# angelocatalani/neural-network-compression

Hardware: AMD Instinct MI355X
Metric: weights/sec through prune+k-means (K=256) (higher is better)
Workload: dtype f32

## Files before the change

neural_network_compression_amd/csrc/nnc_hip.hip:

```cpp
#include "nnc_common.hpp"
#include "nnc_km_shared.hpp"


extern "C" size_t nnc_kmeans_workspace_bytes(int32_t k)
{
    (void)k;
    return sizeof(KmWs) + 256;
}

extern "C" int32_t nnc_fix_shift(float absmax, int64_t n_total)
{
    int L = 1;
    while (((int64_t)1 << L) < n_total && L < 62) L++;
    if (!(absmax > 0.0f) || !std::isfinite(absmax)) return 0;
    int P = 0;
    (void)std::frexp((double)absmax, &P);
    return std::min(28, 62 - L) - P;
}

__device__ __forceinline__ int fix_f32(float v, int Sft)
{
    return (int)rintf(ldexpf(v, Sft));
}

// ... 1156 lines not shown
    if (NNC_FIN_TRACE_PTR && tid == 0) {
        unsigned long long *rt = NNC_FIN_TRACE_PTR;
        const int it = min(ws->st.iter, 63);
        rt[300 + 4 * it] = (unsigned long long)hd->n_empty; rt[301 + 4 * it] = (unsigned long long)hd->nch; rt[302 + 4 * it] = (unsigned long long)hd->slow; rt[303 + 4 * it] = (unsigned long long)ku;
    }
    if (hd->slow || hd->nch > 1024) return 0;
    if constexpr (MASS) {
        if (mass) {
            __shared__ KlMass mass_s;
            return kl_relocate_mass<NT>(xs, n, ws, hd, L, &mass_s, sum_o, cnt_o, k, hd->nch, mean, Sft);
        }
    }
    return kl_relocate<NT>(xs, n, ws, hd, L, sum_o, cnt_o, k, hd->nch, mean, Sft);
}

template <int NT, bool ONEWAVE, bool MASS = false>
__device__ __forceinline__ bool km_finalize_body(KmWs *__restrict__ ws, int mode, int resume, int *gcell, int *hcell, int *ku_out, const bool lazy = false,
                                                 const float *__restrict__ reloc_xs = nullptr, const long long reloc_n = 0, const int k_hint = 0)
{
    static_assert(!ONEWAVE || NT == 64, "the barrier-free form is for a single wave");
#define FIN_SYNC() do { if (ONEWAVE) wave_lds_fence(); else km_lds_barrier(); } while (0)
#define FIN_OR(slot, x) (ONEWAVE ? (int)__any(x) : km_vote_or(&fin_votes[slot], (x)))
#define FIN_AND(slot, x) (ONEWAVE ? (int)__all(x) : !km_vote_or(&fin_votes[slot], !(x)))
#define FIN_COUNT(slot, x) (ONEWAVE ? (int)__popcll(__ballot(x)) : km_vote_count(&fin_votes[slot], (x)))
    __shared__ int fin_votes[8];
    __shared__ long long sum_o[NNC_KMAX];
    __shared__ long long cnt_o[NNC_KMAX];
    __shared__ __align__(16) float cnew[NNC_KMAX];
    __shared__ float cs[NNC_KMAX];
    __shared__ uint16_t so[NNC_KMAX];
    __shared__ float sq[NNC_KMAX];
    __shared__ unsigned long long sh_key;
    __shared__ int ovf_n;
// ... 143 lines not shown
            if (n_empty > 0 && (MASS || n_empty <= KL_RM_MAX) && !resume && reloc_xs && mode == FIN_FROM_SHARDS && lazy && !(st_iter >= 1 && same_counts_now)) {
                __syncthreads();
                if (ftr && tid == 0) { ftr[20] = ftr[0]; ftr[21] = __builtin_amdgcn_s_memrealtime(); }
                const KmTab *tabc = &ws->tab[cur];
                settled = km_finalize_relocate<NT, MASS>(ws, reloc_xs, reloc_n, tabc, cur ? ku1 : ku0, k, cur, sum_o, cnt_o, ws->p.x_mean, Sft) != 0;
                if (settled) { n_empty = 0; settled_event = true; }
                if (settled && ftr && tid == 0) ftr[22] = __builtin_amdgcn_s_memrealtime();
            }
        }
        if (n_empty > 0 && !resume) {
            int tot_empty = 0;
            if (tid == 0) {
                for (int j = 0; j < k; j++) tot_empty += (cnt_o[j] == 0);
                ws->st.paused = 1; ws->st.n_empty = tot_empty;
                if (lazy) ws->tab[cur].n_ovf = 0;
            }
            return false;
        }
        for (int j = tid; j < k; j += NT)
            if (cnt_o[j] > 0) cnew[j] = (float)ldexp((double)sum_o[j] / (double)cnt_o[j], -Sft);
        FIN_SYNC();
        if (n_empty > 0) {
            for (int j = tid; j < k; j += NT)
                atomicMax(&sh_key, ((unsigned long long)cnt_o[j] << 11) | (unsigned long long)(2047 - j));
            FIN_SYNC();
            const int amax = 2047 - (int)(sh_key & 2047ull);
            for (int j = tid; j < k; j += NT)
                if (cnt_o[j] <= 0) {
                    cnew[j] = (amax < j) ? cnew[amax] : (float)ldexp((double)sum_o[amax], -Sft);
                }
// ... 272 lines not shown
    int c = hi_p - lo_p;
    int field = lo_p;
    if (c >= KM_CNT_SAT) {
        c = KM_CNT_SAT;
        const int idx = atomicAdd(n_ovf, 1);
        if (idx < KM_OVF_MAX) { ovf[idx] = (unsigned)lo_p | ((unsigned)hi_p << 16); field = idx; }
        else field = (int)KM_OVF_ALL;
    }
    return (uint16_t)(field | (c << KM_P_BITS));
}

template <int NT, bool FUSED, bool MASS = false>
__device__ __forceinline__ void km_finalize_kernel(KmWs *__restrict__ ws, int mode, int resume,
                                                   nnc_kmeans_status *host_st, unsigned long long *host_ticket,
                                                   unsigned long long ticket, int lazy, const float *__restrict__ reloc_xs,
                                                   long long reloc_n)
{
    __shared__ int gcell[NNC_KMAX], hcell[NNC_KMAX];
    __shared__ int fin_go, fin_kc[2], fin_novf;
    __shared__ int fin_asked;
    const int tid = threadIdx.x;
    const int cond = lazy & 2;
    const int k_hint = lazy >> 8;
    lazy &= 1;
    if (cond) {
        if (tid == 0) fin_asked = ws->wide;
        __syncthreads();
    }
    if (cond && !fin_asked) {
    } else if (FUSED) {
        const int glog2 = ws->glog2;
// ... 1 lines not shown
        __syncthreads();
        if (tid < NT) {
            const bool built = km_finalize_body<NT, FUSED>(ws, mode, resume, gcell, hcell, fin_kc, lazy != 0, reloc_xs, reloc_n, k_hint);
            if (tid == 0) __hip_atomic_store(&fin_go, (built && !lazy) ? 1 : 2, __ATOMIC_RELEASE, __HIP_MEMORY_SCOPE_WORKGROUP);
        }
        int go;
        while ((go = __hip_atomic_load(&fin_go, __ATOMIC_ACQUIRE, __HIP_MEMORY_SCOPE_WORKGROUP)) == 0) __builtin_amdgcn_s_sleep(1);
        if (go == 1) {
            KmTab *tab = &ws->tab[fin_kc[1]];
            const int G = 1 << glog2, ku = fin_kc[0];
            for (int g = tid; g < G; g += KM_THREADS) tab->cell[g] = km_cell_entry(g, G, ku, gcell, hcell, &fin_novf, tab->ovf);
            __syncthreads();
            if (tid == 0) tab->n_ovf = fin_novf;
        }
    } else {
        km_finalize_body<NT, false, MASS>(ws, mode, resume, gcell, hcell, fin_kc, lazy != 0, reloc_xs, reloc_n, k_hint);
    }
    if (cond && fin_asked) {
        __syncthreads();
        if (tid == 0) { ws->wide = 0; ws->kl_budget = ws->kl_budget - 1; ws->kl_stats[4] += 1; }
    }
    if (host_st) {
        __syncthreads();
        if (tid == 0) {
            *host_st = ws->st;
            __threadfence_system();
            *reinterpret_cast<volatile unsigned long long *>(host_ticket) = ticket;
        }
    }
}

template <int NT, bool FUSED, bool MASS = false>
__global__ __launch_bounds__(FUSED ? KM_THREADS : NT) void k_finalize(KmWs *__restrict__ ws, int mode, int resume,
                                                                      nnc_kmeans_status *host_st, unsigned long long *host_ticket,
                                                                      unsigned long long ticket, int lazy, const float *__restrict__ reloc_xs,
                                                                      long long reloc_n)
{
    km_finalize_kernel<NT, FUSED, MASS>(ws, mode, resume, host_st, host_ticket, ticket, lazy, reloc_xs, reloc_n);
}

__global__ __launch_bounds__(KM_THREADS) void k_fit_small(const float *__restrict__ xs, long long n, KmWs *__restrict__ ws,
                                                         const long long *__restrict__ pblk, int iters, nnc_kmeans_status *host_st,
                                                         unsigned long long *host_ticket, unsigned long long ticket)
{
    __shared__ int gcell[NNC_KMAX], hcell[NNC_KMAX];
    __shared__ int fin_kc[2];
    const int tid = threadIdx.x, lane = tid & 63, wv = uni_i(tid >> 6);
    const float mean = ws->p.x_mean;
    const int Sft = ws->p.fix_shift;
    for (int it = 0; it < iters; it++) {
        if (ws->st.done | ws->st.paused) break;
        const KmTab *tab = &ws->tab[ws->cur];
        const int ku = ws->bnd.ku;
// ... 103 lines not shown
    return p->prefix_dev && p->n > 0 && p->n == p->n_total && km_fused(p) && (reinterpret_cast<uintptr_t>(x) & 15) == 0;
}

static int km_ensure_cells(KmWs *w, const nnc_kmeans_params *p, int which, void *stream)
{
    if (!p->prefix_dev) return NNC_OK;
    hipLaunchKernelGGL(k_cells_prepare, dim3(1), dim3(1), 0, S(stream), w, which);
    LAUNCHCHK("k_cells_prepare");
    hipLaunchKernelGGL(k_cells, dim3(KM_GMAX / KM_THREADS), dim3(KM_THREADS), 0, S(stream), w, (nnc_kmeans_status *)nullptr,
                       (unsigned long long *)nullptr, 0ull, 1, which);
    LAUNCHCHK("k_cells");
    return NNC_OK;
}

int km_launch_finalize(KmWs *w, const nnc_kmeans_params *p, int mode, int resume, void *stream, void *host_mapped,
                       uint64_t ticket, bool cond, const float *reloc_xs)
{
    const int k = p ? p->k : 0;
    bool fused = false;
    if (p && mode != FIN_PACK_ONLY) fused = km_fused(p);
    const bool lazy = p && p->prefix_dev;
    const bool cells = mode != FIN_PACK_ONLY && !fused && !lazy;
    unsigned char *hb = reinterpret_cast<unsigned char *>(host_mapped);
    nnc_kmeans_status *hs = reinterpret_cast<nnc_kmeans_status *>(hb);
    unsigned long long *ht = reinterpret_cast<unsigned long long *>(hb ? hb + sizeof(nnc_kmeans_status) : nullptr);
    nnc_kmeans_status *fs = cells ? nullptr : hs;
#define KM_LAUNCH_FIN(NT, FUSED, THREADS) NNC_LAUNCH_PROF(NNC_PROF_FINALIZE, (k_finalize<NT, FUSED>), dim3(1), dim3(THREADS), 0, S(stream), w, mode, resume, fs, ht, (unsigned long long)ticket, (lazy ? 1 : 0) | (cond ? 2 : 0) | (k > 0 ? k << 8 : 0), reloc_xs, (long long)(p ? p->n : 0))
#define KM_LAUNCH_FIN_MASS(NT, THREADS) NNC_LAUNCH_PROF(NNC_PROF_FINALIZE, (k_finalize<NT, false, true>), dim3(1), dim3(THREADS), 0, S(stream), w, mode, resume, fs, ht, (unsigned long long)ticket, (lazy ? 1 : 0) | (cond ? 2 : 0) | (k > 0 ? k << 8 : 0), reloc_xs, (long long)(p ? p->n : 0))
    const bool mass = p && (p->flags & NNC_KM_MASS_IN_PLACE) && reloc_xs && !fused && k > 64;
    if (fused) KM_LAUNCH_FIN(64, true, KM_THREADS);
    else if (k > 0 && k <= 64) KM_LAUNCH_FIN(64, false, 64);
    else if (k > 0 && k <= 256) { if (mass) KM_LAUNCH_FIN_MASS(256, 256); else KM_LAUNCH_FIN(256, false, 256); }
    else { if (mass) KM_LAUNCH_FIN_MASS(KM_THREADS, KM_THREADS); else KM_LAUNCH_FIN(KM_THREADS, false, KM_THREADS); }
#undef KM_LAUNCH_FIN_MASS
#undef KM_LAUNCH_FIN
    LAUNCHCHK("k_finalize");
    if (cells) {
        hipLaunchKernelGGL(k_cells, dim3(KM_GMAX / KM_THREADS), dim3(KM_THREADS), 0, S(stream), w, hs, ht, (unsigned long long)ticket, 0, 0);
        LAUNCHCHK("k_cells");
    }
    return NNC_OK;
}

// ... 719 lines not shown
    km_relocate_body(ws, keys, nkeys, &lds);
}

extern "C" int nnc_kmeans_relocate(void *ws, const int64_t *keys_sorted_dev, int32_t nkeys, void *stream)
{
    if (!ws || !keys_sorted_dev || nkeys < 0) return fail(NNC_EINVAL, "nnc_kmeans_relocate: bad argument");
    if (nkeys == 0) return NNC_OK;
    hipLaunchKernelGGL(k_relocate, dim3(1), dim3(KM_THREADS), 0, S(stream), reinterpret_cast<KmWs *>(ws),
                       reinterpret_cast<const long long *>(keys_sorted_dev), nkeys);
    LAUNCHCHK("k_relocate");
    return NNC_OK;
}

struct KmWin { long long start; int len; int off; };

template <bool MAXOP>
__device__ __forceinline__ void block_scan2(long long &a0, long long &a1, long long *wave_tot)
{
    const int tid = threadIdx.x, lane = tid & 63, wv = tid >> 6;
    auto op = [](long long x, long long y) -> long long { return MAXOP ? (x > y ? x : y) : x + y; };
    a1 = op(a0, a1);
    long long s = a1;
    for (int off = 1; off < 64; off <<= 1) {
        const long long t = __shfl_up(s, off);
        if (lane >= off) s = op(s, t);
    }
    if (lane == 63) wave_tot[wv] = s;
    __syncthreads();
    long long pre = 0;
    for (int w = 0; w < wv; w++) pre = op(pre, wave_tot[w]);
// ... 9 lines not shown
#define KM_RELOC_WMIN 64
#endif
#define KM_SURV_MAX 2048
#define KM_SURV_SMALL 384

__device__ __forceinline__ bool km_spec_decide(const KmWs *__restrict__ ws, long long n, int spec_wmax, int *W_out)
{
    const int done = ws->st.done, paused = ws->st.paused, it = ws->st.iter, same = ws->st.same_counts, ne = ws->st.n_empty;
    long long w = KM_RELOC_WMIN;
    while (w < ne) w *= 2;
    if (W_out) *W_out = (int)w;
    return !done && paused == 1 && !(it >= 1 && same) && ne >= 1 && w <= spec_wmax && 2 * w <= n;
}

__device__ __forceinline__ void km_reloc_windows_body(const float *__restrict__ xs, long long n, KmWs *__restrict__ ws, int W, long long cap,
                                                      KmWin *__restrict__ win, int *__restrict__ meta, unsigned *__restrict__ hist0, int spec_wmax)
{
    if (spec_wmax > 0) {
        const bool go = km_spec_decide(ws, n, spec_wmax, &W);
        if (threadIdx.x == 0) ws->spec_go = go ? 1 : 0;
        if (!go) return;
    }
    if (hist0) for (int i = threadIdx.x; i < 4096; i += KM_THREADS) hist0[i] = 0u;
    __shared__ long long bnd[2 * KM_THREADS + 2];
    __shared__ long long wst[2 * KM_THREADS], wen[2 * KM_THREADS];
    __shared__ long long wave_tot[KM_THREADS / 64];
    const int tid = threadIdx.x;
    const KmTab *tab = &ws->tab[ws->cur];
    const int kt = tab->ku, k = ws->p.k;
    const float mean = ws->p.x_mean;
    const int i0 = 2 * tid, i1 = 2 * tid + 1;
    long long a0 = (i0 < kt) ? ws->partials_local[k + tab->orig[i0]] : 0;
    long long a1 = (i1 < kt) ? ws->partials_local[k + tab->orig[i1]] : 0;
    block_scan2<false>(a0, a1, wave_tot);
    if (tid == 0) bnd[0] = 0;
    bnd[i0 + 1] = a0; bnd[i1 + 1] = a1;
    __syncthreads();
    const int nwin = kt + 1;
    const int bad = (bnd[kt] != n) ? 1 : 0;
    if (bad) {
        for (int j = tid; j < nwin; j += KM_THREADS) { KmWin w; w.start = 0; w.len = 0; w.off = 0; win[j] = w; }
        if (tid == 0) { meta[0] = 0; meta[1] = nwin; meta[2] = 1; meta[3] = W; }
        return;
    }
    for (int j = tid; j < 2 * KM_THREADS; j += KM_THREADS) {
        long long st = 0, en = 0;
        if (j < nwin) {
            long long b = bnd[j];
// ... 27 lines not shown
    const long long len0 = l0, len1 = l1;
    block_scan2<false>(l0, l1, wave_tot);
    if (i0 < nwin) { KmWin w; w.start = s0; w.len = (int)len0; w.off = l0 <= cap ? (int)(l0 - len0) : 0; win[i0] = w; }
    if (i1 < nwin) { KmWin w; w.start = s1; w.len = (int)len1; w.off = l1 <= cap ? (int)(l1 - len1) : 0; win[i1] = w; }
    if (tid == (nwin - 1) / 2) {
        const long long total = ((nwin - 1) & 1) ? l1 : l0;
        const int over = total > cap ? 1 : 0;
        meta[0] = over ? 0 : (int)total; meta[1] = nwin; meta[2] = bad | over; meta[3] = W;
    }
}

__global__ __launch_bounds__(KM_THREADS) void k_reloc_windows(const float *__restrict__ xs, long long n, KmWs *__restrict__ ws,
                                                              int W, long long cap, KmWin *__restrict__ win, int *__restrict__ meta,
                                                              unsigned *__restrict__ hist0 = nullptr, int spec_wmax = 0)
{
    if (spec_wmax > 0 && threadIdx.x == 0 && km_spec_decide(ws, n, spec_wmax, nullptr)) ws->tab[ws->cur].n_ovf = 0;
    km_reloc_windows_body(xs, n, ws, W, cap, win, meta, hist0, spec_wmax);
}

__global__ __launch_bounds__(KM_THREADS) void k_reloc_head(const float *__restrict__ xs, long long n, KmWs *__restrict__ ws, long long cap,
                                                           KmWin *__restrict__ win, int *__restrict__ meta, unsigned *__restrict__ hist0, int spec_wmax)
{
    if (blockIdx.x == gridDim.x - 1) {
        km_reloc_windows_body(xs, n, ws, 0, cap, win, meta, hist0, spec_wmax);
    } else {
        if (!km_spec_decide(ws, n, spec_wmax, nullptr)) return;
        km_cells_body(ws, nullptr, nullptr, 0ull, 1, 0, 0, (int)blockIdx.x);
    }
}

__global__ __launch_bounds__(256) void k_reloc_fill(const float *__restrict__ xs, const KmWin *__restrict__ win,
                                                    const int *__restrict__ meta, float *__restrict__ cand_x, long long cap)
{
    const int lane = threadIdx.x & 63;
    const int wave = (int)((blockIdx.x * blockDim.x + threadIdx.x) >> 6), nwaves = (int)((gridDim.x * blockDim.x) >> 6);
    const int nwin = meta[1];
    const long long total = meta[0];
    if (!meta[2])
        for (int j = wave; j < nwin; j += nwaves) {
            const KmWin w = win[j];
            for (int i = lane; i < w.len; i += 64) cand_x[w.off + i] = xs[w.start + i];
        }
    if (blockIdx.x == 0 && threadIdx.x < 4 && total + threadIdx.x < cap) cand_x[total + threadIdx.x] = 0.0f;
}

__global__ __launch_bounds__(KM_THREADS) void k_reloc_dist(const float *__restrict__ xs, const KmWin *__restrict__ win,
                                                           const int *__restrict__ meta, float *__restrict__ cand_x,
                                                           float *__restrict__ cand_d, long long cap, const KmWs *__restrict__ ws,
                                                           unsigned *__restrict__ hist0, int spec = 0)
{
    extern __shared__ __align__(16) unsigned char smem[];
    __shared__ unsigned h0_s[4096];
    if (spec && !ws->spec_go) return;
    for (int i = threadIdx.x; i < 4096; i += KM_THREADS) h0_s[i] = 0u;
    if (meta[2]) {
        if (blockIdx.x == 0 && threadIdx.x < 4 && threadIdx.x < cap) { cand_x[threadIdx.x] = 0.0f; cand_d[threadIdx.x] = 0.0f; }
        return;
    }
    const int k = ws->p.k, glog2 = ws->glog2;
    const int G = 1 << glog2, kp = (k + 7) & ~7;
    const KmTab *__restrict__ tab = &ws->tab[ws->cur];
    const int kt = tab->ku;
    uint16_t *cell_s = reinterpret_cast<uint16_t *>(smem);
    float4 *pair_s = reinterpret_cast<float4 *>(smem + ((size_t)2 << glog2));
    float *cval_s = reinterpret_cast<float *>(smem + ((size_t)2 << glog2) + (size_t)kp * 16);
    uint16_t *orig_s = reinterpret_cast<uint16_t *>(smem + ((size_t)2 << glog2) + (size_t)kp * 20);
    const size_t off = (((size_t)2 << glog2) + (size_t)kp * 22 + 15) & ~(size_t)15;
    unsigned *ovf_s = reinterpret_cast<unsigned *>(smem + off);
    {
        const uint4 *src = reinterpret_cast<const uint4 *>(tab->cell);
        uint4 *dst = reinterpret_cast<uint4 *>(cell_s);
        for (int i = threadIdx.x; i < (G >> 3); i += KM_THREADS) dst[i] = src[i];
        for (int i = threadIdx.x; i < kt; i += KM_THREADS) {
            const float2 a = tab->cand[i];
            const float2 b = (i + 1 < kt) ? tab->cand[i + 1] : a;
            pair_s[i] = make_float4(a.x, a.y, b.x, b.y);
            cval_s[i] = a.x;
            orig_s[i] = tab->orig[i];
        }
        const int novf = min(tab->n_ovf, KM_OVF_MAX);
        for (int i = threadIdx.x; i < novf; i += KM_THREADS) ovf_s[i] = tab->ovf[i];
    }
    __syncthreads();
    KmCtx c;
    c.cell_s = cell_s; c.pair_s = pair_s; c.cval_s = cval_s; c.orig_s = orig_s; c.ovf_s = ovf_s; c.sum_s = nullptr; c.cnt_s = nullptr;
    c.mean = ws->p.x_mean; c.lo = ws->p.lo; c.inv = ws->inv;
    c.Sft = ws->p.fix_shift; c.gmax = G - 1; c.k = kt; c.rlog2 = 0; c.rep = 0;
    const int nwin = meta[1];
    const long long total = meta[0];
    int *woff_s = reinterpret_cast<int *>(smem + off + KM_OVF_MAX * 4);
    for (int j = threadIdx.x; j < nwin; j += KM_THREADS) woff_s[j] = win[j].off;
    __syncthreads();
    for (long long i = (long long)blockIdx.x * KM_THREADS + threadIdx.x; i < total; i += (long long)gridDim.x * KM_THREADS) {
        int l = 0, h = nwin - 1;
        while (l < h) { const int m = (l + h + 1) >> 1; if (woff_s[m] <= (int)i) l = m; else h = m - 1; }
        KmWin w = win[l];
        while (w.len == 0 || (int)i - w.off >= w.len) { l--; w = win[l]; }
        const float xv[1] = {xs[w.start + ((int)i - w.off)]};
        float xc[1];
        int p[1];
        km_resolve<1>(c, xv, xc, p);
        const float dd = xc[0] - cval_s[p[0]];
        const float dv = dd * dd;
        cand_x[i] = xv[0];
        cand_d[i] = dv;
        atomicAdd(&h0_s[(__float_as_uint(dv) >> 19) & 4095u], 1u);
    }
    __syncthreads();
    for (int i = threadIdx.x; i < 4096; i += KM_THREADS)
        if (h0_s[i]) atomicAdd(&hist0[i], h0_s[i]);
    if (blockIdx.x == 0 && threadIdx.x < 4 && total + threadIdx.x < cap) { cand_x[total + threadIdx.x] = 0.0f; cand_d[total + threadIdx.x] = 0.0f; }
}

__device__ __forceinline__ void km_reloc_select_body(KmWs *__restrict__ ws, const float *__restrict__ cand_x,
                                                     const float *__restrict__ cand_d, const KmWin *__restrict__ win,
                                                     const int *__restrict__ meta, int n_empty, long long *__restrict__ keys_out,
                                                     int do_relocate, const unsigned *__restrict__ hist0, int spec)
{
    if (spec) {
// ... 213 lines not shown

__global__ __launch_bounds__(KM_THREADS) void k_reloc_select(KmWs *__restrict__ ws, const float *__restrict__ cand_x,
                                                             const float *__restrict__ cand_d, const KmWin *__restrict__ win,
                                                             const int *__restrict__ meta, int n_empty, long long *__restrict__ keys_out,
                                                             int do_relocate, const unsigned *__restrict__ hist0, int spec)
{
    km_reloc_select_body(ws, cand_x, cand_d, win, meta, n_empty, keys_out, do_relocate, hist0, spec);
}

__global__ __launch_bounds__(KM_THREADS) void k_reloc_select_finalize(KmWs *__restrict__ ws, const float *__restrict__ cand_x,
                                                                      const float *__restrict__ cand_d, const KmWin *__restrict__ win,
                                                                      const int *__restrict__ meta, long long *__restrict__ keys_out,
                                                                      const unsigned *__restrict__ hist0, nnc_kmeans_status *host_st,
                                                                      unsigned long long *host_ticket, unsigned long long ticket, int lazy)
{
    km_reloc_select_body(ws, cand_x, cand_d, win, meta, 0, keys_out, 1, hist0, 1);
    __syncthreads();
    __builtin_amdgcn_fence(__ATOMIC_ACQUIRE, "agent");
    km_finalize_kernel<KM_THREADS, false, false>(ws, FIN_FROM_PARTIALS, 2, host_st, host_ticket, ticket, lazy, nullptr, 0);
}

static std::atomic<int> g_reloc_dist_attr[NNC_MAX_DEVICES];
static int km_reloc_windows_dist(const float *x_sorted, void *ws, const nnc_kmeans_params *p, int32_t window, float *cand_x,
                                 float *cand_d, int64_t cap, void *win_dev, int32_t *meta_dev, unsigned *hist0, void *stream)
{
    int glog2, rlog2;
    km_defaults(p, &glog2, &rlog2);
    const size_t lds = km_lds_bytes(p->k, glog2, rlog2, false) + (NNC_KMAX + 2) * sizeof(int);
    if (lds > 128 * 1024) return fail(NNC_EINVAL, "relocation: search tables too large for the candidate kernel");
    if (!g_reloc_dist_attr[current_device()].load(std::memory_order_acquire)) {
        HIPCHK(hipFuncSetAttribute(reinterpret_cast<const void *>(&k_reloc_dist), hipFuncAttributeMaxDynamicSharedMemorySize, 128 * 1024));
        g_reloc_dist_attr[current_device()].store(1, std::memory_order_release);
    }
    {
        int rc = km_ensure_cells(reinterpret_cast<KmWs *>(ws), p, 0, stream);
        if (rc) return rc;
    }
    NNC_LAUNCH_PROF(NNC_PROF_RELOC, k_reloc_windows, dim3(1), dim3(KM_THREADS), 0, S(stream), x_sorted, (long long)p->n,
                       reinterpret_cast<KmWs *>(ws), (int)window, (long long)cap,
                       reinterpret_cast<KmWin *>(win_dev), reinterpret_cast<int *>(meta_dev), hist0, 0);
    LAUNCHCHK("k_reloc_windows");
    const int grid = (int)std::max<int64_t>(1, std::min<int64_t>(128, (2 * (int64_t)window * (p->k + 1) + KM_THREADS - 1) / KM_THREADS));
    NNC_LAUNCH_PROF(NNC_PROF_RELOC, k_reloc_dist, dim3(grid), dim3(KM_THREADS), lds, S(stream), x_sorted, reinterpret_cast<const KmWin *>(win_dev),
                       reinterpret_cast<const int *>(meta_dev), cand_x, cand_d, (long long)cap, reinterpret_cast<const KmWs *>(ws), hist0, 0);
    LAUNCHCHK("k_reloc_dist");
    return NNC_OK;
}

extern "C" int nnc_kmeans_reloc_candidates(const float *x_sorted, void *ws, const nnc_kmeans_params *p, int32_t window,
                                           float *cand_x_dev, int64_t cap, void *win_dev, int32_t *meta_dev, void *stream)
{
    int rc = km_check(ws, p, "nnc_kmeans_reloc_candidates");
    if (rc) return rc;
    if (!x_sorted || !cand_x_dev || !win_dev || !meta_dev || window < 1) return fail(NNC_EINVAL, "nnc_kmeans_reloc_candidates: bad argument");
    if (cap < 2 * (int64_t)window * (p->k + 1) || cap > 0x7FFFFFFF) return fail(NNC_ENOSPACE, "nnc_kmeans_reloc_candidates: cap must be in [2 * window * (k + 1), 2^31)");
    NNC_LAUNCH_PROF(NNC_PROF_RELOC, k_reloc_windows, dim3(1), dim3(KM_THREADS), 0, S(stream), x_sorted, (long long)p->n,
                       reinterpret_cast<KmWs *>(ws), (int)window, (long long)cap,
                       reinterpret_cast<KmWin *>(win_dev), reinterpret_cast<int *>(meta_dev), (unsigned *)nullptr, 0);
// ... 23 lines not shown
                       reinterpret_cast<const KmWin *>(win_dev), reinterpret_cast<const int *>(meta_dev), (int)n_empty,
                       reinterpret_cast<long long *>(keys_out_dev), 1, (const unsigned *)nullptr, 0);
    LAUNCHCHK("k_reloc_select");
    return NNC_OK;
}


extern "C" int32_t nnc_kmeans_reloc_window(int64_t n, int32_t n_empty)
{
    int64_t w = KM_RELOC_WMIN;
    while (w < n_empty) w *= 2;
    if (n_empty < 1 || w > 1024 || 2 * w > n) return 0;
    return (int32_t)w;
}

static int64_t reloc_cap(int32_t k, int32_t window) { return 8 * (int64_t)window * (k + 1); }

extern "C" size_t nnc_kmeans_reloc_scratch_bytes(int32_t k, int32_t window)
{
    if (k < 1 || window < 1) return 0;
    const size_t cap = (size_t)reloc_cap(k, window);
    return 2 * reloc_align(cap * 4) + reloc_align(16 * (size_t)(k + 2)) + reloc_align(16) + reloc_align(8 * (size_t)NNC_KMAX) + reloc_align(4096 * 4);
}

extern "C" int nnc_kmeans_relocate_windowed(const float *x_sorted, void *ws, const nnc_kmeans_params *p, int32_t n_empty,
                                            void *scratch_dev, size_t scratch_bytes, void *stream)
{
    int rc = km_check(ws, p, "nnc_kmeans_relocate_windowed");
    if (rc) return rc;
    const int32_t window = nnc_kmeans_reloc_window(p->n, n_empty);
    if (window == 0) return fail(NNC_EINVAL, "nnc_kmeans_relocate_windowed: not applicable (nnc_kmeans_reloc_window() == 0)");
// ... 4 lines not shown
    unsigned char *b = reinterpret_cast<unsigned char *>(scratch_dev);
    float *cand_x = reinterpret_cast<float *>(b); b += reloc_align((size_t)cap * 4);
    float *cand_d = reinterpret_cast<float *>(b); b += reloc_align((size_t)cap * 4);
    void *win = b; b += reloc_align(16 * (size_t)(p->k + 2));
    int32_t *meta = reinterpret_cast<int32_t *>(b); b += reloc_align(16);
    int64_t *keys = reinterpret_cast<int64_t *>(b); b += reloc_align(8 * (size_t)NNC_KMAX);
    unsigned *hist0 = reinterpret_cast<unsigned *>(b);
    if ((rc = km_reloc_windows_dist(x_sorted, ws, p, window, cand_x, cand_d, cap, win, meta, hist0, stream))) return rc;
    NNC_LAUNCH_PROF(NNC_PROF_RELOC, k_reloc_select, dim3(1), dim3(KM_THREADS), 0, S(stream), reinterpret_cast<KmWs *>(ws), cand_x, cand_d,
                       reinterpret_cast<const KmWin *>(win), reinterpret_cast<const int *>(meta), (int)n_empty,
                       reinterpret_cast<long long *>(keys), 1, (const unsigned *)hist0, 0);
    LAUNCHCHK("k_reloc_select");
    return km_launch_finalize(reinterpret_cast<KmWs *>(ws), p, FIN_FROM_PARTIALS, 1, stream);
}

#define KM_SPEC_WMAX 256
static int km_launch_spec_reloc(const float *x_sorted, KmWs *w, const nnc_kmeans_params *p, void *scratch_dev, void *stream,
                                void *host_mapped, uint64_t ticket)
{
    const int32_t wmax = KM_SPEC_WMAX;
    const int64_t cap = reloc_cap(p->k, wmax);
    unsigned char *b = reinterpret_cast<unsigned char *>(scratch_dev);
    float *cand_x = reinterpret_cast<float *>(b); b += reloc_align((size_t)cap * 4);
    float *cand_d = reinterpret_cast<float *>(b); b += reloc_align((size_t)cap * 4);
    KmWin *win = reinterpret_cast<KmWin *>(b); b += reloc_align(16 * (size_t)(p->k + 2));
    int *meta = reinterpret_cast<int *>(b); b += reloc_align(16);
    long long *keys = reinterpret_cast<long long *>(b); b += reloc_align(8 * (size_t)NNC_KMAX);
    unsigned *hist0 = reinterpret_cast<unsigned *>(b);
    int glog2, rlog2;
    km_defaults(p, &glog2, &rlog2);
    const size_t lds = km_lds_bytes(p->k, glog2, rlog2, false) + (NNC_KMAX + 2) * sizeof(int);
    if (lds > 128 * 1024) return fail(NNC_EINVAL, "relocation: search tables too large for the candidate kernel");
    if (!g_reloc_dist_attr[current_device()].load(std::memory_order_acquire)) {
        HIPCHK(hipFuncSetAttribute(reinterpret_cast<const void *>(&k_reloc_dist), hipFuncAttributeMaxDynamicSharedMemorySize, 128 * 1024));
        g_reloc_dist_attr[current_device()].store(1, std::memory_order_release);
    }
    NNC_LAUNCH_PROF(NNC_PROF_RELOC, k_reloc_head, dim3(KM_GMAX / KM_THREADS + 1), dim3(KM_THREADS), 0, S(stream), x_sorted, (long long)p->n, w, (long long)cap, win, meta,
                       hist0, (int)wmax);
    LAUNCHCHK("k_reloc_head");
    const int grid = (int)std::max<int64_t>(1, std::min<int64_t>(128, (2 * (int64_t)64 * (p->k + 1) + KM_THREADS - 1) / KM_THREADS));
    NNC_LAUNCH_PROF(NNC_PROF_RELOC, k_reloc_dist, dim3(grid), dim3(KM_THREADS), lds, S(stream), x_sorted, (const KmWin *)win, (const int *)meta, cand_x, cand_d, (long long)cap,
                       reinterpret_cast<const KmWs *>(w), hist0, 1);
    LAUNCHCHK("k_reloc_dist");
#ifndef KM_CHAIN_FIVE
    if (p->k > 256 && !km_fused(p) && p->prefix_dev) {
        unsigned char *hb = reinterpret_cast<unsigned char *>(host_mapped);
        NNC_LAUNCH_PROF(NNC_PROF_RELOC, k_reloc_select_finalize, dim3(1), dim3(KM_THREADS), 0, S(stream), w, (const float *)cand_x, (const float *)cand_d, (const KmWin *)win,
                        (const int *)meta, keys, (const unsigned *)hist0, reinterpret_cast<nnc_kmeans_status *>(hb),
                        reinterpret_cast<unsigned long long *>(hb ? hb + sizeof(nnc_kmeans_status) : nullptr), (unsigned long long)ticket, 1 | (p->k << 8));
        LAUNCHCHK("k_reloc_select_finalize");
        return NNC_OK;
    }
#endif
    NNC_LAUNCH_PROF(NNC_PROF_RELOC, k_reloc_select, dim3(1), dim3(KM_THREADS), 0, S(stream), w, (const float *)cand_x, (const float *)cand_d, (const KmWin *)win, (const int *)meta, 0, keys, 1, (const unsigned *)hist0, 1);
    LAUNCHCHK("k_reloc_select");
    return km_launch_finalize(w, p, FIN_FROM_PARTIALS, 2, stream, host_mapped, ticket);
}


int nnc_wait_ticket_(void *host_ticket, uint64_t ticket, void *stream)
{
    return km_wait_ticket(reinterpret_cast<volatile unsigned long long *>(host_ticket), (unsigned long long)ticket, S(stream));
}
int km_wait_ticket(volatile unsigned long long *word, unsigned long long ticket, hipStream_t stream)
{
    unsigned long long spins = 0;
    bool synced = false;
    auto t0 = std::chrono::steady_clock::now();
    while (__atomic_load_n(word, __ATOMIC_ACQUIRE) != ticket) {
// ... 33 lines not shown
    int nwin = 0, nrel_seen = status_out->n_relocated, nunp_seen = status_out->n_unproven;
    int nip_seen = status_out->n_in_place;
    if (!spec_ok) { nrel_seen = 0; nunp_seen = 0; nip_seen = 0; }
    double s_prev = -1.0, s_last = -1.0;
    int i_prev = 0, i_last = 0;
    KmWs *w = reinterpret_cast<KmWs *>(ws);
    for (;;) {
        const uint64_t ticket = ++(*ticket_io);
        unsigned char *sl = hb + (ticket & 1) * slot;
        if (lloyd) {
            if ((rc = km_set_lds_attr())) return rc;
            for (int i = 0; i < batch; i++) {
                const bool last = i == batch - 1;
                if ((rc = km_launch_lloyd_round(x_iter, w, &p, first_launch ? p.max_iter : -1, stream, (last && !spec) ? sl : nullptr, ticket, spec ? 1 : 0))) return rc;
                first_launch = false;
                if (spec && (rc = km_launch_spec_reloc(x_iter, w, &p, reloc_scratch_dev, stream, last ? sl : nullptr, ticket))) return rc;
            }
        } else if (spec) {
            if ((rc = km_set_lds_attr())) return rc;
            for (int i = 0; i < batch; i++) {
                if ((rc = km_launch_accumulate(x_iter, w, &p, stream))) return rc;
                if ((rc = km_launch_finalize(w, &p, FIN_FROM_SHARDS, 0, stream, nullptr, 0, false, x_iter))) return rc;
                if ((rc = km_launch_spec_reloc(x_iter, w, &p, reloc_scratch_dev, stream, i == batch - 1 ? sl : nullptr, ticket))) return rc;
            }
        } else {
            const int lag = (!one_launch && batch >= 4) ? KM_FIT_LAG : 0;
            if ((rc = km_iterate_publish_(x_iter, ws, &p, batch, sl, ticket, stream, spec_ok, lag))) return rc;
        }
        if ((rc = km_wait_ticket(reinterpret_cast<volatile unsigned long long *>(sl + sizeof(nnc_kmeans_status)), ticket, S(stream)))) return rc;
        const nnc_kmeans_status st = *reinterpret_cast<const nnc_kmeans_status *>(sl);
        *status_out = st;
        const int dev_events = spec_ok ? st.n_relocated - nrel_seen : 0;
        const int chain_events = dev_events - (spec_ok ? st.n_in_place - nip_seen : 0);
        nrel_seen = st.n_relocated;
        nip_seen = st.n_in_place;
        nwin += dev_events;
        nwin += spec_ok ? st.n_unproven - nunp_seen : 0;
        nunp_seen = st.n_unproven;
// ... 172 lines not shown
```

neural_network_compression_amd/csrc/nnc_km_shared.hpp:

```cpp
#pragma once
#define KM_THREADS 1024
#define KL_RKEYS 16384
#define KM_NSHARD 8
#define KM_GMAX 32768
#define KM_CNT_SAT 31
#define KM_P_BITS 11
#define KM_P_MASK 2047u
#define KM_OVF_MAX 1024
#define KM_OVF_ALL 2047u
#define KM_FUSE_GLOG2 11
#define KM_FUSE_KMAX 64
#ifndef KM_RING
#define KM_RING 4
#endif

struct KmTab {
    float2 cand[NNC_KMAX];
    uint16_t orig[NNC_KMAX];
    uint16_t perm[NNC_KMAX];
    uint32_t ovf[KM_OVF_MAX];
    int32_t n_ovf;
    int32_t ku;
    int32_t pad_[2];
    uint16_t cell[KM_GMAX];
// ... 39 lines not shown
#define FIN_FROM_PARTIALS 2
#define FIN_PACK_ONLY 3

__device__ __forceinline__ int uni_i(int v) { return __builtin_amdgcn_readfirstlane(v); }
__device__ __forceinline__ long long uni_ll(long long v)
{
    const unsigned lo = (unsigned)__builtin_amdgcn_readfirstlane((int)(unsigned)(v & 0xFFFFFFFFll));
    const unsigned hi = (unsigned)__builtin_amdgcn_readfirstlane((int)(unsigned)((unsigned long long)v >> 32));
    return (long long)(((unsigned long long)hi << 32) | lo);
}

int km_check(void *ws, const nnc_kmeans_params *p, const char *who);
int km_set_lds_attr();
int km_launch_accumulate(const float *x, KmWs *w, const nnc_kmeans_params *p, void *stream, int which = 0);
int km_launch_finalize(KmWs *w, const nnc_kmeans_params *p, int mode, int resume, void *stream, void *host_mapped = nullptr,
                       uint64_t ticket = 0, bool cond = false, const float *reloc_xs = nullptr);
int km_wait_ticket(volatile unsigned long long *word, unsigned long long ticket, hipStream_t stream);
static inline size_t reloc_align(size_t b) { return (b + 255) & ~(size_t)255; }
```

Before: 9.943 billion.

## Fold speculative relocation head into finalize and simplify candidate distance kernel

```diff
diff --git a/neural_network_compression_amd/csrc/nnc_hip.hip b/neural_network_compression_amd/csrc/nnc_hip.hip
--- a/neural_network_compression_amd/csrc/nnc_hip.hip
+++ b/neural_network_compression_amd/csrc/nnc_hip.hip
@@ -1194,9 +1194,13 @@
     return kl_relocate<NT>(xs, n, ws, hd, L, sum_o, cnt_o, k, hd->nch, mean, Sft);
 }
 
+__device__ __noinline__ void km_pause_head(KmWs *__restrict__ ws, const float *__restrict__ xs, const long long n, void *scratch,
+                                           const long long *cnt_by_orig, const int st_iter, const int same_counts);
+
 template <int NT, bool ONEWAVE, bool MASS = false>
 __device__ __forceinline__ bool km_finalize_body(KmWs *__restrict__ ws, int mode, int resume, int *gcell, int *hcell, int *ku_out, const bool lazy = false,
-                                                 const float *__restrict__ reloc_xs = nullptr, const long long reloc_n = 0, const int k_hint = 0)
+                                                 const float *__restrict__ reloc_xs = nullptr, const long long reloc_n = 0, const int k_hint = 0,
+                                                 void *chain = nullptr)
 {
     static_assert(!ONEWAVE || NT == 64, "the barrier-free form is for a single wave");
 #define FIN_SYNC() do { if (ONEWAVE) wave_lds_fence(); else km_lds_barrier(); } while (0)
@@ -1370,6 +1374,9 @@
                 for (int j = 0; j < k; j++) tot_empty += (cnt_o[j] == 0);
                 ws->st.paused = 1; ws->st.n_empty = tot_empty;
                 if (lazy) ws->tab[cur].n_ovf = 0;
+            }
+            if constexpr (NT == KM_THREADS && !ONEWAVE && !MASS) {
+                if (chain) km_pause_head(ws, reloc_xs, reloc_n, chain, cnt_o, st_iter, same_counts_now);
             }
             return false;
         }
@@ -1672,7 +1679,7 @@
 __device__ __forceinline__ void km_finalize_kernel(KmWs *__restrict__ ws, int mode, int resume,
                                                    nnc_kmeans_status *host_st, unsigned long long *host_ticket,
                                                    unsigned long long ticket, int lazy, const float *__restrict__ reloc_xs,
-                                                   long long reloc_n)
+                                                   long long reloc_n, void *chain = nullptr)
 {
     __shared__ int gcell[NNC_KMAX], hcell[NNC_KMAX];
     __shared__ int fin_go, fin_kc[2], fin_novf;
@@ -1704,7 +1711,11 @@
             if (tid == 0) tab->n_ovf = fin_novf;
         }
     } else {
-        km_finalize_body<NT, false, MASS>(ws, mode, resume, gcell, hcell, fin_kc, lazy != 0, reloc_xs, reloc_n, k_hint);
+        km_finalize_body<NT, false, MASS>(ws, mode, resume, gcell, hcell, fin_kc, lazy != 0, reloc_xs, reloc_n, k_hint, chain);
+    }
+    if (resume == 2) {
+        __syncthreads();
+        if (tid == 0) ws->spec_go = 0;
     }
     if (cond && fin_asked) {
         __syncthreads();
@@ -1724,9 +1735,9 @@
 __global__ __launch_bounds__(FUSED ? KM_THREADS : NT) void k_finalize(KmWs *__restrict__ ws, int mode, int resume,
                                                                       nnc_kmeans_status *host_st, unsigned long long *host_ticket,
                                                                       unsigned long long ticket, int lazy, const float *__restrict__ reloc_xs,
-                                                                      long long reloc_n)
-{
-    km_finalize_kernel<NT, FUSED, MASS>(ws, mode, resume, host_st, host_ticket, ticket, lazy, reloc_xs, reloc_n);
+                                                                      long long reloc_n, void *chain)
+{
+    km_finalize_kernel<NT, FUSED, MASS>(ws, mode, resume, host_st, host_ticket, ticket, lazy, reloc_xs, reloc_n, chain);
 }
 
 __global__ __launch_bounds__(KM_THREADS) void k_fit_small(const float *__restrict__ xs, long long n, KmWs *__restrict__ ws,
@@ -1860,7 +1871,7 @@
 }
 
 int km_launch_finalize(KmWs *w, const nnc_kmeans_params *p, int mode, int resume, void *stream, void *host_mapped,
-                       uint64_t ticket, bool cond, const float *reloc_xs)
+                       uint64_t ticket, bool cond, const float *reloc_xs, void *chain_scratch)
 {
     const int k = p ? p->k : 0;
     bool fused = false;
@@ -1871,8 +1882,8 @@
     nnc_kmeans_status *hs = reinterpret_cast<nnc_kmeans_status *>(hb);
     unsigned long long *ht = reinterpret_cast<unsigned long long *>(hb ? hb + sizeof(nnc_kmeans_status) : nullptr);
     nnc_kmeans_status *fs = cells ? nullptr : hs;
-#define KM_LAUNCH_FIN(NT, FUSED, THREADS) NNC_LAUNCH_PROF(NNC_PROF_FINALIZE, (k_finalize<NT, FUSED>), dim3(1), dim3(THREADS), 0, S(stream), w, mode, resume, fs, ht, (unsigned long long)ticket, (lazy ? 1 : 0) | (cond ? 2 : 0) | (k > 0 ? k << 8 : 0), reloc_xs, (long long)(p ? p->n : 0))
-#define KM_LAUNCH_FIN_MASS(NT, THREADS) NNC_LAUNCH_PROF(NNC_PROF_FINALIZE, (k_finalize<NT, false, true>), dim3(1), dim3(THREADS), 0, S(stream), w, mode, resume, fs, ht, (unsigned long long)ticket, (lazy ? 1 : 0) | (cond ? 2 : 0) | (k > 0 ? k << 8 : 0), reloc_xs, (long long)(p ? p->n : 0))
+#define KM_LAUNCH_FIN(NT, FUSED, THREADS) NNC_LAUNCH_PROF(NNC_PROF_FINALIZE, (k_finalize<NT, FUSED>), dim3(1), dim3(THREADS), 0, S(stream), w, mode, resume, fs, ht, (unsigned long long)ticket, (lazy ? 1 : 0) | (cond ? 2 : 0) | (k > 0 ? k << 8 : 0), reloc_xs, (long long)(p ? p->n : 0), (void *)(NT == KM_THREADS ? chain_scratch : nullptr))
+#define KM_LAUNCH_FIN_MASS(NT, THREADS) NNC_LAUNCH_PROF(NNC_PROF_FINALIZE, (k_finalize<NT, false, true>), dim3(1), dim3(THREADS), 0, S(stream), w, mode, resume, fs, ht, (unsigned long long)ticket, (lazy ? 1 : 0) | (cond ? 2 : 0) | (k > 0 ? k << 8 : 0), reloc_xs, (long long)(p ? p->n : 0), (void *)nullptr)
     const bool mass = p && (p->flags & NNC_KM_MASS_IN_PLACE) && reloc_xs && !fused && k > 64;
     if (fused) KM_LAUNCH_FIN(64, true, KM_THREADS);
     else if (k > 0 && k <= 64) KM_LAUNCH_FIN(64, false, 64);
@@ -2622,6 +2633,24 @@
 
 struct KmWin { long long start; int len; int off; };
 
+#define KM_SPEC_WMAX 256
+__host__ __device__ static inline long long reloc_cap(int k, int window) { return 8 * (long long)window * (k + 1); }
+struct KmSpecScratch { float *cand_x, *cand_d; KmWin *win; int *meta; long long *keys; unsigned *hist0; long long cap; };
+__host__ __device__ static inline KmSpecScratch km_spec_scratch(void *scratch_dev, int k)
+{
+    auto al = [](size_t b) { return (b + 255) & ~(size_t)255; };
+    KmSpecScratch sc;
+    sc.cap = reloc_cap(k, KM_SPEC_WMAX);
+    unsigned char *b = reinterpret_cast<unsigned char *>(scratch_dev);
+    sc.cand_x = reinterpret_cast<float *>(b); b += al((size_t)sc.cap * 4);
+    sc.cand_d = reinterpret_cast<float *>(b); b += al((size_t)sc.cap * 4);
+    sc.win = reinterpret_cast<KmWin *>(b); b += al(16 * (size_t)(k + 2));
+    sc.meta = reinterpret_cast<int *>(b); b += al(16);
+    sc.keys = reinterpret_cast<long long *>(b); b += al(8 * (size_t)NNC_KMAX);
+    sc.hist0 = reinterpret_cast<unsigned *>(b);
+    return sc;
+}
+
 template <bool MAXOP>
 __device__ __forceinline__ void block_scan2(long long &a0, long long &a1, long long *wave_tot)
 {
@@ -2661,7 +2690,8 @@
 }
 
 __device__ __forceinline__ void km_reloc_windows_body(const float *__restrict__ xs, long long n, KmWs *__restrict__ ws, int W, long long cap,
-                                                      KmWin *__restrict__ win, int *__restrict__ meta, unsigned *__restrict__ hist0, int spec_wmax)
+                                                      KmWin *__restrict__ win, int *__restrict__ meta, unsigned *__restrict__ hist0, int spec_wmax,
+                                                      const long long *cnt_by_orig = nullptr)
 {
     if (spec_wmax > 0) {
         const bool go = km_spec_decide(ws, n, spec_wmax, &W);
@@ -2677,8 +2707,9 @@
     const int kt = tab->ku, k = ws->p.k;
     const float mean = ws->p.x_mean;
     const int i0 = 2 * tid, i1 = 2 * tid + 1;
-    long long a0 = (i0 < kt) ? ws->partials_local[k + tab->orig[i0]] : 0;
-    long long a1 = (i1 < kt) ? ws->partials_local[k + tab->orig[i1]] : 0;
+    const long long *cnt = cnt_by_orig ? cnt_by_orig : ws->partials_local + k;
+    long long a0 = (i0 < kt) ? cnt[tab->orig[i0]] : 0;
+    long long a1 = (i1 < kt) ? cnt[tab->orig[i1]] : 0;
     block_scan2<false>(a0, a1, wave_tot);
     if (tid == 0) bnd[0] = 0;
     bnd[i0 + 1] = a0; bnd[i1 + 1] = a1;
@@ -2736,19 +2767,28 @@
                                                               int W, long long cap, KmWin *__restrict__ win, int *__restrict__ meta,
                                                               unsigned *__restrict__ hist0 = nullptr, int spec_wmax = 0)
 {
-    if (spec_wmax > 0 && threadIdx.x == 0 && km_spec_decide(ws, n, spec_wmax, nullptr)) ws->tab[ws->cur].n_ovf = 0;
     km_reloc_windows_body(xs, n, ws, W, cap, win, meta, hist0, spec_wmax);
 }
 
-__global__ __launch_bounds__(KM_THREADS) void k_reloc_head(const float *__restrict__ xs, long long n, KmWs *__restrict__ ws, long long cap,
-                                                           KmWin *__restrict__ win, int *__restrict__ meta, unsigned *__restrict__ hist0, int spec_wmax)
-{
-    if (blockIdx.x == gridDim.x - 1) {
-        km_reloc_windows_body(xs, n, ws, 0, cap, win, meta, hist0, spec_wmax);
-    } else {
-        if (!km_spec_decide(ws, n, spec_wmax, nullptr)) return;
-        km_cells_body(ws, nullptr, nullptr, 0ull, 1, 0, 0, (int)blockIdx.x);
-    }
+__device__ __noinline__ void km_pause_head(KmWs *__restrict__ ws, const float *__restrict__ xs, const long long n, void *scratch,
+                                           const long long *cnt_by_orig, const int st_iter, const int same_counts)
+{
+    __shared__ int ne_s;
+    const int k = ws->p.k;
+    if (threadIdx.x == 0) ne_s = 0;
+    __syncthreads();
+    int e = 0;
+    for (int j = threadIdx.x; j < k; j += KM_THREADS) e += cnt_by_orig[j] == 0;
+    if (e) atomicAdd(&ne_s, e);
+    __syncthreads();
+    const int ne = ne_s;
+    long long w = KM_RELOC_WMIN;
+    while (w < ne) w *= 2;
+    const bool go = !(st_iter >= 1 && same_counts) && ne >= 1 && w <= KM_SPEC_WMAX && 2 * w <= n;
+    if (threadIdx.x == 0) ws->spec_go = go ? 1 : 0;
+    if (!go) return;
+    const KmSpecScratch sc = km_spec_scratch(scratch, k);
+    km_reloc_windows_body(xs, n, ws, (int)w, sc.cap, sc.win, sc.meta, sc.hist0, 0, cnt_by_orig);
 }
 
 __global__ __launch_bounds__(256) void k_reloc_fill(const float *__restrict__ xs, const KmWin *__restrict__ win,
@@ -2771,60 +2811,84 @@
                                                            float *__restrict__ cand_d, long long cap, const KmWs *__restrict__ ws,
                                                            unsigned *__restrict__ hist0, int spec = 0)
 {
-    extern __shared__ __align__(16) unsigned char smem[];
     __shared__ unsigned h0_s[4096];
+    __shared__ float2 cand_s[NNC_KMAX];
+    __shared__ double zrm_s[NNC_KMAX], zlm_s[NNC_KMAX];
+    __shared__ uint16_t orig_s[NNC_KMAX];
+    __shared__ int woff_s[NNC_KMAX + 2];
+    __shared__ double wave_r[KM_THREADS / 64], wave_l[KM_THREADS / 64];
     if (spec && !ws->spec_go) return;
     for (int i = threadIdx.x; i < 4096; i += KM_THREADS) h0_s[i] = 0u;
     if (meta[2]) {
         if (blockIdx.x == 0 && threadIdx.x < 4 && threadIdx.x < cap) { cand_x[threadIdx.x] = 0.0f; cand_d[threadIdx.x] = 0.0f; }
         return;
     }
-    const int k = ws->p.k, glog2 = ws->glog2;
-    const int G = 1 << glog2, kp = (k + 7) & ~7;
     const KmTab *__restrict__ tab = &ws->tab[ws->cur];
-    const int kt = tab->ku;
-    uint16_t *cell_s = reinterpret_cast<uint16_t *>(smem);
-    float4 *pair_s = reinterpret_cast<float4 *>(smem + ((size_t)2 << glog2));
-    float *cval_s = reinterpret_cast<float *>(smem + ((size_t)2 << glog2) + (size_t)kp * 16);
-    uint16_t *orig_s = reinterpret_cast<uint16_t *>(smem + ((size_t)2 << glog2) + (size_t)kp * 20);
-    const size_t off = (((size_t)2 << glog2) + (size_t)kp * 22 + 15) & ~(size_t)15;
-    unsigned *ovf_s = reinterpret_cast<unsigned *>(smem + off);
+    const int kt = min(tab->ku, (int)NNC_KMAX);
+    const float mean = ws->p.x_mean;
+    const int nwin = min(meta[1], (int)NNC_KMAX + 1);
+    const long long total = meta[0];
+    for (int i = threadIdx.x; i < kt; i += KM_THREADS) { cand_s[i] = tab->cand[i]; orig_s[i] = tab->orig[i]; }
+    for (int j = threadIdx.x; j < nwin; j += KM_THREADS) woff_s[j] = win[j].off;
     {
-        const uint4 *src = reinterpret_cast<const uint4 *>(tab->cell);
-        uint4 *dst = reinterpret_cast<uint4 *>(cell_s);
-        for (int i = threadIdx.x; i < (G >> 3); i += KM_THREADS) dst[i] = src[i];
-        for (int i = threadIdx.x; i < kt; i += KM_THREADS) {
-            const float2 a = tab->cand[i];
-            const float2 b = (i + 1 < kt) ? tab->cand[i + 1] : a;
-            pair_s[i] = make_float4(a.x, a.y, b.x, b.y);
-            cval_s[i] = a.x;
-            orig_s[i] = tab->orig[i];
-        }
-        const int novf = min(tab->n_ovf, KM_OVF_MAX);
-        for (int i = threadIdx.x; i < novf; i += KM_THREADS) ovf_s[i] = tab->ovf[i];
-    }
-    __syncthreads();
-    KmCtx c;
-    c.cell_s = cell_s; c.pair_s = pair_s; c.cval_s = cval_s; c.orig_s = orig_s; c.ovf_s = ovf_s; c.sum_s = nullptr; c.cnt_s = nullptr;
-    c.mean = ws->p.x_mean; c.lo = ws->p.lo; c.inv = ws->inv;
-    c.Sft = ws->p.fix_shift; c.gmax = G - 1; c.k = kt; c.rlog2 = 0; c.rep = 0;
-    const int nwin = meta[1];
-    const long long total = meta[0];
-    int *woff_s = reinterpret_cast<int *>(smem + off + KM_OVF_MAX * 4);
-    for (int j = threadIdx.x; j < nwin; j += KM_THREADS) woff_s[j] = win[j].off;
-    __syncthreads();
+        const int lane = threadIdx.x & 63, myw = threadIdx.x >> 6;
+        const int rounds = (kt + KM_THREADS - 1) / KM_THREADS;
+        double carry_r = -INFINITY, carry_l = INFINITY;
+        for (int it = 0; it < rounds; it++) {
+            const int pr = it * KM_THREADS + (int)threadIdx.x, pl = (rounds - 1 - it) * KM_THREADS + (int)threadIdx.x;
+            double a = pr < kt ? tab->zr[pr] : -INFINITY;
+            double b = pl < kt ? tab->zl[pl] : INFINITY;
+            for (int off = 1; off < 64; off <<= 1) {
+                const double oa = __shfl_up(a, off), ob = __shfl_down(b, off);
+                if (lane >= off) a = fmax(a, oa);
+                if (lane + off < 64) b = fmin(b, ob);
+            }
+            if (lane == 63) wave_r[myw] = a;
+            if (lane == 0) wave_l[myw] = b;
+            __syncthreads();
+            double pre = carry_r, totr = carry_r, suf = carry_l, totl = carry_l;
+            for (int w = 0; w < KM_THREADS / 64; w++) {
+                const double rv = wave_r[w], lv = wave_l[w];
+                if (w < myw) pre = fmax(pre, rv);
+                totr = fmax(totr, rv);
+                if (w > myw) suf = fmin(suf, lv);
+                totl = fmin(totl, lv);
+            }
+            if (pr < kt) zrm_s[pr] = fmax(a, pre);
+            if (pl < kt) zlm_s[pl] = fmin(b, suf);
+            carry_r = totr; carry_l = totl;
+            __syncthreads();
+        }
+    }
     for (long long i = (long long)blockIdx.x * KM_THREADS + threadIdx.x; i < total; i += (long long)gridDim.x * KM_THREADS) {
         int l = 0, h = nwin - 1;
         while (l < h) { const int m = (l + h + 1) >> 1; if (woff_s[m] <= (int)i) l = m; else h = m - 1; }
         KmWin w = win[l];
-        while (w.len == 0 || (int)i - w.off >= w.len) { l--; w = win[l]; }
-        const float xv[1] = {xs[w.start + ((int)i - w.off)]};
-        float xc[1];
-        int p[1];
-        km_resolve<1>(c, xv, xc, p);
-        const float dd = xc[0] - cval_s[p[0]];
+        while (l > 0 && (w.len == 0 || (int)i - w.off >= w.len)) { l--; w = win[l]; }
+        const int r = (int)i - w.off;
+        if (r < 0 || r >= w.len) continue;
+        const float xv = xs[w.start + r];
+        const float xc = xv - mean;
+        const double xd = (double)xc;
+        int plo, phi;
+        l = 0; h = kt - 1;
+        while (l < h) { const int m = (l + h) >> 1; if (zrm_s[m] >= xd) h = m; else l = m + 1; }
+        plo = l;
+        l = 0; h = kt - 1;
+        while (l < h) { const int m = (l + h + 1) >> 1; if (zlm_s[m] <= xd) l = m; else h = m - 1; }
+        phi = l;
+        if (phi < plo) { plo = 0; phi = kt - 1; }
+        float2 cc = cand_s[plo];
+        float bestd = cc.y + (-2.0f * (xc * cc.x));
+        int best = plo;
+        for (int q = plo + 1; q <= phi; q++) {
+            const float2 ci = cand_s[q];
+            const float d = ci.y + (-2.0f * (xc * ci.x));
+            if (d < bestd || (d == bestd && orig_s[q] < orig_s[best])) { bestd = d; best = q; }
+        }
+        const float dd = xc - cand_s[best].x;
         const float dv = dd * dd;
-        cand_x[i] = xv[0];
+        cand_x[i] = xv;
         cand_d[i] = dv;
         atomicAdd(&h0_s[(__float_as_uint(dv) >> 19) & 4095u], 1u);
     }
@@ -3068,34 +3132,29 @@
                                                                       const unsigned *__restrict__ hist0, nnc_kmeans_status *host_st,
                                                                       unsigned long long *host_ticket, unsigned long long ticket, int lazy)
 {
+    if (!ws->spec_go) {
+        if (host_st && threadIdx.x == 0) {
+            *host_st = ws->st;
+            __threadfence_system();
+            *reinterpret_cast<volatile unsigned long long *>(host_ticket) = ticket;
+        }
+        return;
+    }
     km_reloc_select_body(ws, cand_x, cand_d, win, meta, 0, keys_out, 1, hist0, 1);
     __syncthreads();
     __builtin_amdgcn_fence(__ATOMIC_ACQUIRE, "agent");
     km_finalize_kernel<KM_THREADS, false, false>(ws, FIN_FROM_PARTIALS, 2, host_st, host_ticket, ticket, lazy, nullptr, 0);
 }
 
-static std::atomic<int> g_reloc_dist_attr[NNC_MAX_DEVICES];
 static int km_reloc_windows_dist(const float *x_sorted, void *ws, const nnc_kmeans_params *p, int32_t window, float *cand_x,
                                  float *cand_d, int64_t cap, void *win_dev, int32_t *meta_dev, unsigned *hist0, void *stream)
 {
-    int glog2, rlog2;
-    km_defaults(p, &glog2, &rlog2);
-    const size_t lds = km_lds_bytes(p->k, glog2, rlog2, false) + (NNC_KMAX + 2) * sizeof(int);
-    if (lds > 128 * 1024) return fail(NNC_EINVAL, "relocation: search tables too large for the candidate kernel");
-    if (!g_reloc_dist_attr[current_device()].load(std::memory_order_acquire)) {
-        HIPCHK(hipFuncSetAttribute(reinterpret_cast<const void *>(&k_reloc_dist), hipFuncAttributeMaxDynamicSharedMemorySize, 128 * 1024));
-        g_reloc_dist_attr[current_device()].store(1, std::memory_order_release);
-    }
-    {
-        int rc = km_ensure_cells(reinterpret_cast<KmWs *>(ws), p, 0, stream);
-        if (rc) return rc;
-    }
     NNC_LAUNCH_PROF(NNC_PROF_RELOC, k_reloc_windows, dim3(1), dim3(KM_THREADS), 0, S(stream), x_sorted, (long long)p->n,
                        reinterpret_cast<KmWs *>(ws), (int)window, (long long)cap,
                        reinterpret_cast<KmWin *>(win_dev), reinterpret_cast<int *>(meta_dev), hist0, 0);
     LAUNCHCHK("k_reloc_windows");
     const int grid = (int)std::max<int64_t>(1, std::min<int64_t>(128, (2 * (int64_t)window * (p->k + 1) + KM_THREADS - 1) / KM_THREADS));
-    NNC_LAUNCH_PROF(NNC_PROF_RELOC, k_reloc_dist, dim3(grid), dim3(KM_THREADS), lds, S(stream), x_sorted, reinterpret_cast<const KmWin *>(win_dev),
+    NNC_LAUNCH_PROF(NNC_PROF_RELOC, k_reloc_dist, dim3(grid), dim3(KM_THREADS), 0, S(stream), x_sorted, reinterpret_cast<const KmWin *>(win_dev),
                        reinterpret_cast<const int *>(meta_dev), cand_x, cand_d, (long long)cap, reinterpret_cast<const KmWs *>(ws), hist0, 0);
     LAUNCHCHK("k_reloc_dist");
     return NNC_OK;
@@ -3149,7 +3208,6 @@
     return (int32_t)w;
 }
 
-static int64_t reloc_cap(int32_t k, int32_t window) { return 8 * (int64_t)window * (k + 1); }
 
 extern "C" size_t nnc_kmeans_reloc_scratch_bytes(int32_t k, int32_t window)
 {
@@ -3184,45 +3242,33 @@
     return km_launch_finalize(reinterpret_cast<KmWs *>(ws), p, FIN_FROM_PARTIALS, 1, stream);
 }
 
-#define KM_SPEC_WMAX 256
+static bool km_spec_head_in_finalize(const nnc_kmeans_params *p) { return p->k > 256 && !km_fused(p) && p->prefix_dev; }
+
 static int km_launch_spec_reloc(const float *x_sorted, KmWs *w, const nnc_kmeans_params *p, void *scratch_dev, void *stream,
-                                void *host_mapped, uint64_t ticket)
-{
-    const int32_t wmax = KM_SPEC_WMAX;
-    const int64_t cap = reloc_cap(p->k, wmax);
-    unsigned char *b = reinterpret_cast<unsigned char *>(scratch_dev);
-    float *cand_x = reinterpret_cast<float *>(b); b += reloc_align((size_t)cap * 4);
-    float *cand_d = reinterpret_cast<float *>(b); b += reloc_align((size_t)cap * 4);
-    KmWin *win = reinterpret_cast<KmWin *>(b); b += reloc_align(16 * (size_t)(p->k + 2));
-    int *meta = reinterpret_cast<int *>(b); b += reloc_align(16);
-    long long *keys = reinterpret_cast<long long *>(b); b += reloc_align(8 * (size_t)NNC_KMAX);
-    unsigned *hist0 = reinterpret_cast<unsigned *>(b);
-    int glog2, rlog2;
-    km_defaults(p, &glog2, &rlog2);
-    const size_t lds = km_lds_bytes(p->k, glog2, rlog2, false) + (NNC_KMAX + 2) * sizeof(int);
-    if (lds > 128 * 1024) return fail(NNC_EINVAL, "relocation: search tables too large for the candidate kernel");
-    if (!g_reloc_dist_attr[current_device()].load(std::memory_order_acquire)) {
-        HIPCHK(hipFuncSetAttribute(reinterpret_cast<const void *>(&k_reloc_dist), hipFuncAttributeMaxDynamicSharedMemorySize, 128 * 1024));
-        g_reloc_dist_attr[current_device()].store(1, std::memory_order_release);
-    }
-    NNC_LAUNCH_PROF(NNC_PROF_RELOC, k_reloc_head, dim3(KM_GMAX / KM_THREADS + 1), dim3(KM_THREADS), 0, S(stream), x_sorted, (long long)p->n, w, (long long)cap, win, meta,
-                       hist0, (int)wmax);
-    LAUNCHCHK("k_reloc_head");
+                                void *host_mapped, uint64_t ticket, bool head_done)
+{
+    const KmSpecScratch sc = km_spec_scratch(scratch_dev, p->k);
+    if (!head_done) {
+        NNC_LAUNCH_PROF(NNC_PROF_RELOC, k_reloc_windows, dim3(1), dim3(KM_THREADS), 0, S(stream), x_sorted, (long long)p->n, w, 0, sc.cap, sc.win, sc.meta,
+                        sc.hist0, (int)KM_SPEC_WMAX);
+        LAUNCHCHK("k_reloc_windows");
+    }
     const int grid = (int)std::max<int64_t>(1, std::min<int64_t>(128, (2 * (int64_t)64 * (p->k + 1) + KM_THREADS - 1) / KM_THREADS));
-    NNC_LAUNCH_PROF(NNC_PROF_RELOC, k_reloc_dist, dim3(grid), dim3(KM_THREADS), lds, S(stream), x_sorted, (const KmWin *)win, (const int *)meta, cand_x, cand_d, (long long)cap,
-                       reinterpret_cast<const KmWs *>(w), hist0, 1);
+    NNC_LAUNCH_PROF(NNC_PROF_RELOC, k_reloc_dist, dim3(grid), dim3(KM_THREADS), 0, S(stream), x_sorted, (const KmWin *)sc.win, (const int *)sc.meta, sc.cand_x, sc.cand_d,
+                    (long long)sc.cap, reinterpret_cast<const KmWs *>(w), sc.hist0, 1);
     LAUNCHCHK("k_reloc_dist");
 #ifndef KM_CHAIN_FIVE
     if (p->k > 256 && !km_fused(p) && p->prefix_dev) {
         unsigned char *hb = reinterpret_cast<unsigned char *>(host_mapped);
-        NNC_LAUNCH_PROF(NNC_PROF_RELOC, k_reloc_select_finalize, dim3(1), dim3(KM_THREADS), 0, S(stream), w, (const float *)cand_x, (const float *)cand_d, (const KmWin *)win,
-                        (const int *)meta, keys, (const unsigned *)hist0, reinterpret_cast<nnc_kmeans_status *>(hb),
+        NNC_LAUNCH_PROF(NNC_PROF_RELOC, k_reloc_select_finalize, dim3(1), dim3(KM_THREADS), 0, S(stream), w, (const float *)sc.cand_x, (const float *)sc.cand_d,
+                        (const KmWin *)sc.win, (const int *)sc.meta, sc.keys, (const unsigned *)sc.hist0, reinterpret_cast<nnc_kmeans_status *>(hb),
                         reinterpret_cast<unsigned long long *>(hb ? hb + sizeof(nnc_kmeans_status) : nullptr), (unsigned long long)ticket, 1 | (p->k << 8));
         LAUNCHCHK("k_reloc_select_finalize");
         return NNC_OK;
     }
 #endif
-    NNC_LAUNCH_PROF(NNC_PROF_RELOC, k_reloc_select, dim3(1), dim3(KM_THREADS), 0, S(stream), w, (const float *)cand_x, (const float *)cand_d, (const KmWin *)win, (const int *)meta, 0, keys, 1, (const unsigned *)hist0, 1);
+    NNC_LAUNCH_PROF(NNC_PROF_RELOC, k_reloc_select, dim3(1), dim3(KM_THREADS), 0, S(stream), w, (const float *)sc.cand_x, (const float *)sc.cand_d, (const KmWin *)sc.win,
+                    (const int *)sc.meta, 0, sc.keys, 1, (const unsigned *)sc.hist0, 1);
     LAUNCHCHK("k_reloc_select");
     return km_launch_finalize(w, p, FIN_FROM_PARTIALS, 2, stream, host_mapped, ticket);
 }
@@ -3286,14 +3332,15 @@
                 const bool last = i == batch - 1;
                 if ((rc = km_launch_lloyd_round(x_iter, w, &p, first_launch ? p.max_iter : -1, stream, (last && !spec) ? sl : nullptr, ticket, spec ? 1 : 0))) return rc;
                 first_launch = false;
-                if (spec && (rc = km_launch_spec_reloc(x_iter, w, &p, reloc_scratch_dev, stream, last ? sl : nullptr, ticket))) return rc;
+                if (spec && (rc = km_launch_spec_reloc(x_iter, w, &p, reloc_scratch_dev, stream, last ? sl : nullptr, ticket, false))) return rc;
             }
         } else if (spec) {
             if ((rc = km_set_lds_attr())) return rc;
             for (int i = 0; i < batch; i++) {
                 if ((rc = km_launch_accumulate(x_iter, w, &p, stream))) return rc;
-                if ((rc = km_launch_finalize(w, &p, FIN_FROM_SHARDS, 0, stream, nullptr, 0, false, x_iter))) return rc;
-                if ((rc = km_launch_spec_reloc(x_iter, w, &p, reloc_scratch_dev, stream, i == batch - 1 ? sl : nullptr, ticket))) return rc;
+                const bool head = km_spec_head_in_finalize(&p);
+                if ((rc = km_launch_finalize(w, &p, FIN_FROM_SHARDS, 0, stream, nullptr, 0, false, x_iter, head ? reloc_scratch_dev : nullptr))) return rc;
+                if ((rc = km_launch_spec_reloc(x_iter, w, &p, reloc_scratch_dev, stream, i == batch - 1 ? sl : nullptr, ticket, head))) return rc;
             }
         } else {
             const int lag = (!one_launch && batch >= 4) ? KM_FIT_LAG : 0;
diff --git a/neural_network_compression_amd/csrc/nnc_km_shared.hpp b/neural_network_compression_amd/csrc/nnc_km_shared.hpp
--- a/neural_network_compression_amd/csrc/nnc_km_shared.hpp
+++ b/neural_network_compression_amd/csrc/nnc_km_shared.hpp
@@ -77,6 +77,6 @@
 int km_set_lds_attr();
 int km_launch_accumulate(const float *x, KmWs *w, const nnc_kmeans_params *p, void *stream, int which = 0);
 int km_launch_finalize(KmWs *w, const nnc_kmeans_params *p, int mode, int resume, void *stream, void *host_mapped = nullptr,
-                       uint64_t ticket = 0, bool cond = false, const float *reloc_xs = nullptr);
+                       uint64_t ticket = 0, bool cond = false, const float *reloc_xs = nullptr, void *chain_scratch = nullptr);
 int km_wait_ticket(volatile unsigned long long *word, unsigned long long ticket, hipStream_t stream);
 static inline size_t reloc_align(size_t b) { return (b + 255) & ~(size_t)255; }
```

New measurement: 9.819 billion. -1.2%, worse.
